# santurini/vsrlab

Hardware: AMD Instinct MI355X
Metric: LR frames/sec fwd+bwd, BasicVSR 4x 540p 7-frame clip, 1->8 MI355X (higher is better)
Workload: dtype bf16; 1 GPU; BasicVSR(mid=64,res_blocks=30,x4) fwd+Charbonnier+bwd+clip+Adam, 540x960->2160x3840, 7-frame clip, 2 clips per GPU (BASELINE configs[1]); clips_per_gpu=2, frames=7, res_blocks=30, parallelism=single GPU, arena=full, train_flow=False, trunk_chains=True

## Files before the change

### vsrlab_amd/csrc/conv_mfma.hip

```cpp
#include <cstdlib>
#include "elt.h"

namespace {

__device__ uint4 g_cm_zero[4];

constexpr int TW = 32;
constexpr int RW = 2;
constexpr int TH = 4 * RW;
constexpr int NTHREADS = 256;

typedef __attribute__((ext_vector_type(4))) unsigned cu32x4_t;
typedef __attribute__((ext_vector_type(8))) unsigned cu32x8_t;
template <typename T> struct RegChunk;
template <> struct RegChunk<bf16_t> { typedef cu32x4_t chunk_t; };
template <> struct RegChunk<float> { typedef cu32x8_t chunk_t; };
__device__ __forceinline__ cu32x4_t reg_chunk3(float a, float b, float c, bf16_t*) {
    union { bf16_t h[8]; cu32x4_t u; } t;
    t.u = cu32x4_t{0u, 0u, 0u, 0u};
    t.h[0] = (bf16_t)a; t.h[1] = (bf16_t)b; t.h[2] = (bf16_t)c;
    return t.u;
}
__device__ __forceinline__ cu32x8_t reg_chunk3(float a, float b, float c, float*) {
    return cu32x8_t{__float_as_uint(a), __float_as_uint(b), __float_as_uint(c), 0u, 0u, 0u, 0u, 0u};
// ... 345 lines not shown
int launch_inst(const ConvArgs& a, hipStream_t st) {
    constexpr int TWH = TW + KS - 1, THH = TH + KS - 1;
    constexpr int CMAX = CA > CB ? CA : CB;
    constexpr int CHB = Elt<T>::CHB;
    constexpr int TPS = conv_taps_per_stage<KS, NSRC>(THH * TWH * (CMAX / 8) * CHB, COUT * (CMAX / 8) * CHB);
    constexpr int LDS = THH * TWH * (CMAX / 8) * CHB + (TPS > 1 ? TPS : 2) * COUT * (CMAX / 8) * CHB;
    static_assert(LDS <= 160 * 1024, "tile does not fit the 160 KiB LDS of a CU");
    auto kern = conv_mfma_kernel<T, KS, NSRC, CA, CB, LP, COUT, EPI>;
    static VsrDevOnce once;
    { const int rc = vsr_set_max_dynamic_lds(once, reinterpret_cast<const void*>(kern), LDS); if (rc != VSR_OK) return rc; }
    dim3 grid(cdiv(a.W, TW), cdiv(a.H, TH), a.N * a.nz);
    hipLaunchKernelGGL(kern, grid, dim3(NTHREADS), LDS, st, a);
    HIP_CHECK_RET(hipGetLastError());
    return VSR_OK;
}

}

#define VSR_CONV_SHAPES(X)                  \
    X(3, 1, 64, 64, false, 64, EPI_NHWC)     \
    X(3, 2, 64, 16, true, 64, EPI_NHWC)      \
    X(3, 1, 16, 16, true, 64, EPI_NHWC)      \
    X(3, 1, 64, 64, false, 32, EPI_PLANAR)   \
    X(3, 4, 64, 64, false, 64, EPI_NHWC)     \
    X(1, 2, 64, 64, false, 64, EPI_NHWC)     \
    X(1, 1, 64, 64, false, 64, EPI_NHWC)     \
    X(7, 1, 16, 16, false, 32, EPI_NHWC)     \
    X(7, 1, 32, 32, false, 64, EPI_NHWC)     \
    X(7, 1, 64, 64, false, 32, EPI_NHWC)     \
    X(7, 1, 32, 32, false, 32, EPI_NHWC)    \
    X(7, 1, 16, 16, false, 32, EPI_PLANAR)   \
     \
    X(3, 1, 16, 16, false, 32, EPI_NHWC)     \
    X(3, 1, 32, 32, false, 32, EPI_NHWC)     \
    X(3, 2, 16, 16, true, 32, EPI_NHWC)      \
    X(3, 2, 32, 16, true, 32, EPI_NHWC)      \
    X(3, 1, 16, 16, true, 32, EPI_NHWC)      \
    X(1, 2, 16, 16, false, 32, EPI_NHWC)     \
    X(1, 2, 32, 32, false, 32, EPI_NHWC)    \
    X(1, 1, 16, 16, false, 32, EPI_NHWC)     \
    X(1, 1, 32, 32, false, 32, EPI_NHWC)    \
    X(3, 4, 16, 16, false, 32, EPI_NHWC)     \
    X(3, 4, 32, 32, false, 32, EPI_NHWC)    \
    X(3, 1, 16, 16, false, 64, EPI_NHWC)     \
    X(3, 1, 32, 32, false, 64, EPI_NHWC)    \
    X(3, 1, 64, 64, false, 32, EPI_NHWC)     \
    X(3, 1, 16, 16, false, 32, EPI_PLANAR)   \
    X(3, 1, 32, 32, false, 32, EPI_PLANAR)

int vsr_launch_conv3x3_c64_persist(const ConvArgs& a, int num_cus, hipStream_t st);
int vsr_launch_c64_to_planar(const ConvArgs& a, hipStream_t st);
int vsr_launch_planar_c64_conv(const ConvArgs& a, hipStream_t st);
int vsr_launch_conv7x7_persist(const ConvArgs& a, int cin, int cop, int epi, int num_cus, hipStream_t st);

static bool vsr_force_generic_conv() { return vsr_env().generic_conv; }

int vsr_launch_conv(int dtype, int ks, int nsrc, int ca, int cb, int last_planar, int cout_t, int epi,
                    const ConvArgs& a, hipStream_t st) {
    if (a.N <= 0 || a.H <= 0 || a.W <= 0 || a.nz < 1 || a.nz > VSR_MAX_Z) return VSR_ERR_BADARG;
    if (dtype == VSR_BF16 && ks == 3 && nsrc == 1 && ca == 64 && cb == 64 && !last_planar && cout_t == 64 && epi == EPI_NHWC &&
        ((a.in_step == 1 && a.src_oy[0] == 0 && a.src_ox[0] == 0 && a.Hs == a.H && a.Ws == a.W) ||
         (a.in_step == 2 && a.Hs == 2 * a.H && a.Ws == 2 * a.W && (unsigned)a.src_oy[0] < 2u && (unsigned)a.src_ox[0] < 2u)) &&
        a.CD == 64 && a.cout_real == 64 &&
        a.src[0] != nullptr && !vsr_force_generic_conv()) {
        const int ps = vsr_launch_conv3x3_c64_persist(a, vsr_num_cus(), st);
        if (ps != VSR_ERR_UNSUPPORTED) return ps;
    }
    if (a.unshuffle) return VSR_ERR_UNSUPPORTED;
    if (dtype == VSR_BF16 && ks == 3 && nsrc == 1 && ca == 64 && cb == 64 && !last_planar && cout_t == 32 && epi == EPI_PLANAR &&
        !vsr_force_generic_conv()) {
        const int ps = vsr_launch_c64_to_planar(a, st);
        if (ps != VSR_ERR_UNSUPPORTED) return ps;
    }
    if (dtype == VSR_BF16 && ks == 3 && nsrc == 1 && last_planar && ca == 16 && cb == 16 && cout_t == 64 && epi == EPI_NHWC && !vsr_force_generic_conv()) {
        const int ps = vsr_launch_planar_c64_conv(a, st);
        if (ps != VSR_ERR_UNSUPPORTED) return ps;
    }
    if (dtype == VSR_BF16 && ks == 7 && nsrc == 1 && ca == cb && !last_planar && !vsr_force_generic_conv()) {
        const int ps = vsr_launch_conv7x7_persist(a, ca, cout_t, epi, vsr_num_cus(), st);
        if (ps != VSR_ERR_UNSUPPORTED) return ps;
    }
#define X(KS, NSRC, CA, CB, LP, COUT, EPI)                                                             \
    if (ks == KS && nsrc == NSRC && ca == CA && cb == CB && (last_planar != 0) == LP && cout_t == COUT && epi == EPI) { \
        if (dtype == VSR_BF16) return launch_inst<bf16_t, KS, NSRC, CA, CB, LP, COUT, EPI>(a, st);    \
        if (dtype == VSR_F32) return launch_inst<float, KS, NSRC, CA, CB, LP, COUT, EPI>(a, st);      \
        return VSR_ERR_BADARG;                                                                        \
    }
    VSR_CONV_SHAPES(X)
#undef X
    return VSR_ERR_UNSUPPORTED;
}
```

### vsrlab_amd/csrc/elementwise.hip

```cpp
#include "elt.h"
#include "kernels.h"

namespace {

__device__ __forceinline__ float warp_coord(float base, float flow, int dim) {
    const float d = (float)(dim - 1 > 1 ? dim - 1 : 1);
    const float g = 2.0f * (base + flow) / d - 1.0f;
    return (g + 1.0f) * 0.5f * (float)(dim - 1);
}

struct WarpSample {
    int x0, y0;
    float wx0, wx1, wy0, wy1;
    float px, py;
    bool in_x, in_y;
};
__device__ __forceinline__ void warp_sample_at(float px, float py, WarpSample& s) {
    const float fx0 = floorf(px), fy0 = floorf(py);
    s.x0 = (int)fx0; s.y0 = (int)fy0;
    s.wx1 = px - fx0; s.wy1 = py - fy0; s.wx0 = 1.f - s.wx1; s.wy0 = 1.f - s.wy1;
}
__device__ __forceinline__ bool warp_floor_fits(float px, float py) {
    return !(fabsf(floorf(px)) > 1e9f || fabsf(floorf(py)) > 1e9f);
}
__device__ __forceinline__ WarpSample warp_sample(int x, int y, float flow_x, float flow_y, int H, int W, int border) {
    WarpSample s;
    float px = warp_coord((float)x, flow_x, W);
    float py = warp_coord((float)y, flow_y, H);
    s.px = px; s.py = py;
    s.in_x = !border || (px >= 0.f && px <= (float)(W - 1)); s.in_y = !border || (py >= 0.f && py <= (float)(H - 1));
    if (border) { px = fminf(fmaxf(px, 0.f), (float)(W - 1)); py = fminf(fmaxf(py, 0.f), (float)(H - 1)); }
    warp_sample_at(px, py, s);
    return s;
}
__device__ __forceinline__ float grad_gate_open(float p, int dim) { return (p <= 0.f || p >= (float)(dim - 1)) ? 0.f : 1.f; }

struct WarpTap { int xi, yi; float wgt; };
__device__ __forceinline__ WarpTap warp_tap(const WarpSample& s, int t) {
    WarpTap p;
    p.xi = s.x0 + (t & 1); p.yi = s.y0 + (t >> 1);
    p.wgt = ((t & 1) ? s.wx1 : s.wx0) * ((t >> 1) ? s.wy1 : s.wy0);
    return p;
}
#define TAP_IN_IMAGE(p, H, W) ((p).xi >= 0 && (p).xi < (W) && (p).yi >= 0 && (p).yi < (H))

template <typename T>
__global__ void warp_fwd_kernel(const T* __restrict__ in, const float* __restrict__ flow, T* __restrict__ out,
                                int N, int H, int W, int C, long long flow_nstride, int border) {
    typedef typename Elt<T>::chunk_t chunk_t;
    const int CP = C / 8;
    const long long total = (long long)N * H * W * CP;
    for (long long idx = (long long)blockIdx.x * blockDim.x + threadIdx.x; idx < total; idx += (long long)gridDim.x * blockDim.x) {
        const int c = (int)(idx % CP);
        const long long pix = idx / CP;
        const int x = (int)(pix % W);
        const int y = (int)((pix / W) % H);
        const int n = (int)(pix / ((long long)W * H));
        const float* fp = flow + (long long)n * flow_nstride + (long long)y * W + x;
        const WarpSample s = warp_sample(x, y, fp[0], fp[(long long)H * W], H, W, border);
        float accv[8];
#pragma unroll
        for (int j = 0; j < 8; ++j) accv[j] = 0.f;
        const T* img = in + (long long)n * pm_image_elems(H, W, C);
#pragma unroll
        for (int t = 0; t < 4; ++t) {
            const WarpTap p = warp_tap(s, t);
            if (TAP_IN_IMAGE(p, H, W)) {
                float f[8];
                unpack8(*reinterpret_cast<const chunk_t*>(img + pm_off(p.yi, p.xi, c, W, C)), f);
#pragma unroll
                for (int j = 0; j < 8; ++j) accv[j] += f[j] * p.wgt;
            }
        }
        chunk_t o;
        pack8(accv, o);
        *reinterpret_cast<chunk_t*>(out + (long long)n * pm_image_elems(H, W, C) + pm_off(y, x, c, W, C)) = o;
    }
}

template <typename T>
__global__ void warp_bwd_kernel(const T* __restrict__ dout, const float* __restrict__ flow, float* __restrict__ dacc,
                                int N, int H, int W, int C, long long flow_nstride, int border) {
    const long long total = (long long)N * H * W * C;
    for (long long idx = (long long)blockIdx.x * blockDim.x + threadIdx.x; idx < total; idx += (long long)gridDim.x * blockDim.x) {
        const int c = (int)(idx % C);
        const long long pix = idx / C;
        const int x = (int)(pix % W);
        const int y = (int)((pix / W) % H);
        const int n = (int)(pix / ((long long)W * H));
        const float* fp = flow + (long long)n * flow_nstride + (long long)y * W + x;
        const WarpSample s = warp_sample(x, y, fp[0], fp[(long long)H * W], H, W, border);
        const float g = (float)dout[(long long)n * pm_image_elems(H, W, C) + pm_off(y, x, c >> 3, W, C) + (c & 7)];
        float* img = dacc + (long long)n * H * W * C;
#pragma unroll
        for (int t = 0; t < 4; ++t) {
            const WarpTap p = warp_tap(s, t);
            if (TAP_IN_IMAGE(p, H, W)) atomicAdd(img + ((long long)p.yi * W + p.xi) * C + c, g * p.wgt);
        }
    }
}

constexpr int GR = 5;
constexpr int GTH = 8, GTW = 32, GCAP = 8;
constexpr int GHH = GTH + 2 * GR, GHW = GTW + 2 * GR;
constexpr double FAR_FX = 17592186044416.0;
constexpr int FAR_BAD = 0x40000000;

__device__ __forceinline__ bool flow_is_far(float fx, float fy) {
    return !(fabsf(fx) <= (float)(GR - 1) && fabsf(fy) <= (float)(GR - 1));
}

template <typename T, int C>
__global__ __launch_bounds__(256) void warp_bwd_gather_kernel(const T* __restrict__ dout, const float* __restrict__ flow, const T* __restrict__ dtop,
                                                              long long* __restrict__ S, const int* __restrict__ far_count, T* __restrict__ out,
                                                              int N, int H, int W, long long flow_nstride) {
    constexpr int CP = C / 8, PPP = 256 / CP;
    typedef typename Elt<T>::chunk_t chunk_t;
    __shared__ float2 pos[GHH * GHW];
    __shared__ unsigned short hit_src[256 * GCAP];
    __shared__ float hit_w[256 * GCAP];
    __shared__ int hit_n[256];
    const int tid = threadIdx.x;
    const int ntx = cdiv(W, GTW), nty = cdiv(H, GTH);
    const int tile = blockIdx.x;
    const int n = tile / (ntx * nty), tr = tile - n * ntx * nty;
    const int ty0 = (tr / ntx) * GTH, tx0 = (tr % ntx) * GTW;
    const float* fbase = flow + (long long)n * flow_nstride;
    const long long img = (long long)n * pm_image_elems(H, W, C);
    for (int i = tid; i < GHH * GHW; i += 256) {
// ... 563 lines not shown
    float4* d4 = reinterpret_cast<float4*>(dsr);
    for (long long i = (long long)blockIdx.x * blockDim.x + threadIdx.x; i < n4; i += (long long)gridDim.x * blockDim.x) {
        const float4 a = s4[i], b = h4[i];
        float4 o;
        float d, r;
        d = a.x - b.x; r = sqrtf(d * d + eps); local += r; o.x = scale * d / r;
        d = a.y - b.y; r = sqrtf(d * d + eps); local += r; o.y = scale * d / r;
        d = a.z - b.z; r = sqrtf(d * d + eps); local += r; o.z = scale * d / r;
        d = a.w - b.w; r = sqrtf(d * d + eps); local += r; o.w = scale * d / r;
        d4[i] = o;
    }
    if (!vec) {
        for (long long i = (long long)blockIdx.x * blockDim.x + threadIdx.x; i < n; i += (long long)gridDim.x * blockDim.x) {
            const float d = sr[i] - hr[i];
            const float r = sqrtf(d * d + eps);
            local += r;
            dsr[i] = scale * d / r;
        }
    } else if (blockIdx.x == 0 && threadIdx.x < (int)(n & 3)) {
        const long long i = (n4 << 2) + threadIdx.x;
        const float d = sr[i] - hr[i];
        const float r = sqrtf(d * d + eps);
        local += r;
        dsr[i] = scale * d / r;
    }
    for (int o = 32; o > 0; o >>= 1) local += __shfl_down(local, o, 64);
    if ((threadIdx.x & 63) == 0) red[threadIdx.x >> 6] = local;
    __syncthreads();
    if (threadIdx.x == 0) partial[blockIdx.x] = ((red[0] + red[1]) + (red[2] + red[3])) * scale;
}
__global__ void charbonnier_sum_kernel(const float* __restrict__ partial, int nblocks, float* __restrict__ loss) {
    __shared__ float red[256];
    float s = 0.f;
    for (int i = threadIdx.x; i < nblocks; i += 256) s += partial[i];
    red[threadIdx.x] = s;
    __syncthreads();
    for (int o = 128; o > 0; o >>= 1) {
        if (threadIdx.x < o) red[threadIdx.x] += red[threadIdx.x + o];
        __syncthreads();
    }
    if (threadIdx.x == 0) loss[0] = red[0];
}

}

#define DISPATCH_T(dtype, CALL)                              \
    if ((dtype) == VSR_BF16) { typedef bf16_t T; CALL; }     \
    else if ((dtype) == VSR_F32) { typedef float T; CALL; }  \
    else return VSR_ERR_BADARG;

int vsr_launch_warp_fwd(int dtype, const void* in, const float* flow, void* out, int N, int H, int W, int C,
                        long long flow_nstride, hipStream_t st, int border) {
    if (C % 8) return VSR_ERR_BADARG;
    const long long total = (long long)N * H * W * (C / 8);
    DISPATCH_T(dtype, hipLaunchKernelGGL(warp_fwd_kernel<T>, dim3(grid_for(total)), dim3(256), 0, st, (const T*)in, flow, (T*)out, N, H, W, C, flow_nstride, border));
    HIP_CHECK_RET(hipGetLastError());
    return VSR_OK;
}

int vsr_launch_warp_bwd(int dtype, const void* dout, const float* flow, float* dacc, int N, int H, int W, int C,
                        long long flow_nstride, hipStream_t st, int border) {
    const long long total = (long long)N * H * W * C;
    DISPATCH_T(dtype, hipLaunchKernelGGL(warp_bwd_kernel<T>, dim3(grid_for(total)), dim3(256), 0, st, (const T*)dout, flow, dacc, N, H, W, C, flow_nstride, border));
    HIP_CHECK_RET(hipGetLastError());
    return VSR_OK;
}

template <int C>
static int warp_bwd_gather_c(int dtype, const void* dout, const float* flow, const void* dtop, long long* S, int* far_count, void* out,
                             int N, int H, int W, long long flow_nstride, hipStream_t st) {
    const long long npix = (long long)N * H * W;
    const int tiles = N * cdiv(H, GTH) * cdiv(W, GTW);
    long long gb = (npix + 255) / 256;
    if (gb > 256 * 16) gb = 256 * 16;
    if (gb < 1) gb = 1;
    DISPATCH_T(dtype, hipLaunchKernelGGL((warp_bwd_far_kernel<T, C>), dim3((int)gb), dim3(256), 0, st, (const T*)dout, flow, S, far_count, N, H, W, flow_nstride));
    DISPATCH_T(dtype, hipLaunchKernelGGL((warp_bwd_gather_kernel<T, C>), dim3(tiles), dim3(256), 0, st, (const T*)dout, flow, (const T*)dtop, S,
                                         (const int*)far_count, (T*)out, N, H, W, flow_nstride));
    HIP_CHECK_RET(hipGetLastError());
    return VSR_OK;
}
int vsr_launch_warp_bwd_gather(int dtype, const void* dout, const float* flow, const void* dtop, long long* S, int* far_count, void* out,
                               int N, int H, int W, int C, long long flow_nstride, hipStream_t st) {
    if (!dout || !flow || !S || !far_count || !out) return VSR_ERR_BADARG;
    if (C == 64) return warp_bwd_gather_c<64>(dtype, dout, flow, dtop, S, far_count, out, N, H, W, flow_nstride, st);
    if (C == 32) return warp_bwd_gather_c<32>(dtype, dout, flow, dtop, S, far_count, out, N, H, W, flow_nstride, st);
    if (C == 16) return warp_bwd_gather_c<16>(dtype, dout, flow, dtop, S, far_count, out, N, H, W, flow_nstride, st);
    return VSR_ERR_UNSUPPORTED;
}

int vsr_launch_add_cast(int dtype, const void* a, const float* s, void* out, int N, int H, int W, int C, hipStream_t st) {
    const long long total = (long long)N * H * W * (C / 8);
    DISPATCH_T(dtype, hipLaunchKernelGGL(add_cast_kernel<T>, dim3(grid_for(total)), dim3(256), 0, st, (const T*)a, s, (T*)out, N, H, W, C));
    HIP_CHECK_RET(hipGetLastError());
    return VSR_OK;
}

int vsr_launch_planar_to_pm(int dtype, const float* in, void* out, int N, int Cin, int H, int W, int C, hipStream_t st) {
    const long long total = (long long)N * H * W * C;
    DISPATCH_T(dtype, hipLaunchKernelGGL(planar_to_pm_kernel<T>, dim3(grid_for(total)), dim3(256), 0, st, in, (T*)out, N, Cin, H, W, C));
    HIP_CHECK_RET(hipGetLastError());
    return VSR_OK;
}

int vsr_launch_pm_to_planar(int dtype, const void* in, float* out, int N, int Cout, int H, int W, int C, hipStream_t st) {
    const long long total = (long long)N * Cout * H * W;
    DISPATCH_T(dtype, hipLaunchKernelGGL(pm_to_planar_kernel<T>, dim3(grid_for(total)), dim3(256), 0, st, (const T*)in, out, N, Cout, H, W, C));
    HIP_CHECK_RET(hipGetLastError());
// ... 121 lines not shown
```

### vsrlab_amd/csrc/engine.hip

```cpp
#include <vector>
#include "recipes.h"
#include "spynet_engine.h"

namespace {

struct Plan {
    VsrBasicVSRDesc d = {};
    int C = 64, CO = 64;
    bool sb = false;
    bool bwd = false, flowgrad = false;
    bool diet = false;
    int rb = 0, n = 0, t = 0, h = 0, w = 0, dtype = VSR_F32;
    int scale = 4, ups = 2;
    bool unsh = false;
    size_t es = 4;
    size_t px1 = 0;
    size_t s_elems = 0;
    size_t stem_w[2] = {}, stem_wd[2] = {}, stem_b[2] = {};
    std::vector<size_t> blk_w[2], blk_wd[2], blk_b[2];
    size_t point_w = 0, point_wd = 0, point_b = 0;
    size_t up_w[2] = {}, up_wd[2] = {}, up_b[2] = {};
    size_t last0_w = 0, last0_wd = 0, last0_b = 0, last2_w = 0, last2_wd = 0, last2_b = 0;
    SpyPlan spy;
    size_t flows = 0;
// ... 243 lines not shown
              chain_off(p.blk_w[dir][2 * b]), chain_off(p.blk_b[dir][2 * b]), CHAIN_RELU};
        ChainLayer& l2 = a.layer[2 * b + 1];
        l2 = {chain_off(p.aoff(dir, i, b)), chain_off(p.xoff(dir, i, b + 1)), chain_off(p.xoff(dir, i, b)), 0xffffffffu, 0xffffffffu,
              chain_off(p.blk_w[dir][2 * b + 1]), chain_off(p.blk_b[dir][2 * b + 1]), CHAIN_SKIP};
    }
    return chain_launch(a, c.st);
}
int trunk_chain_backward(const Ctx& c, const Plan& p, int dir, int i) {
    ChainArgs a = {};
    a.base = c.ws; a.sync = (unsigned*)c.at(p.chain_sync[dir]); a.N = p.n; a.H = p.h; a.W = p.w;
    int L = 0;
    for (int b = p.rb - 1; b >= 0; --b) {
        a.layer[L++] = {chain_off(p.dxoff(dir, i, b + 1)), chain_off(p.g1off(dir, i, b)), 0xffffffffu, chain_off(p.sboff(dir, i, b)), 0xffffffffu,
                        chain_off(p.blk_wd[dir][2 * b + 1]), 0xffffffffu, CHAIN_MASK};
        if (b > 0)
            a.layer[L++] = {chain_off(p.g1off(dir, i, b)), chain_off(p.dxoff(dir, i, b)), chain_off(p.dxoff(dir, i, b + 1)), 0xffffffffu, 0xffffffffu,
                            chain_off(p.blk_wd[dir][2 * b]), 0xffffffffu, CHAIN_SKIP};
    }
    a.nlayers = L;
    return chain_launch(a, c.st);
}

int trunk_forward(const Ctx& c, const Plan& p, int dir, int i, const void* warped, const float* lrs) {
    const int n = p.n, h = p.h, w = p.w, rb = p.rb;
    void* x = p.bwd ? c.at(p.xoff(dir, i, 0)) : c.at(p.feat[dir][i]);
    {
        CK(c.stem(true, warped, lrs + (size_t)i * 3 * h * w, (long long)p.t * 3 * h * w, c.at(p.stem_w[dir]), c.fat(p.stem_b[dir]), x, ACT_LEAKY, 0.f, n, h, w));
        if (p.sb) CK(vsr_launch_sign_bits_c64(x, c.at(p.SBX0[dir][i]), n, h, w, c.st));
    }
    if (chain_on(p)) return trunk_chain_forward(c, p, dir, i);
    for (int b = 0; b < rb; ++b) {
        void* act = p.bwd ? c.at(p.aoff(dir, i, b)) : c.at(p.scratchA[dir]);
        void* xn = p.bwd ? c.at(p.xoff(dir, i, b + 1)) : x;
        CK(c.conv(3, x, c.at(p.blk_w[dir][2 * b]), c.fat(p.blk_b[dir][2 * b]), act, ACT_RELU, nullptr, nullptr, 0, n, h, w,
                    p.sb ? c.at(p.sboff(dir, i, b)) : nullptr));
        CK(c.conv(3, act, c.at(p.blk_w[dir][2 * b + 1]), c.fat(p.blk_b[dir][2 * b + 1]), xn, ACT_NONE, x, nullptr, 0, n, h, w));
        x = xn;
    }
    return VSR_OK;
}

int last0_forward(const Ctx& c, const Plan& p, int i, void* sign_out) {
    const int S = p.scale;
    if (p.C == 64)
        return c.conv(3, c.at(p.U1[i]), c.at(p.last0_w), c.fat(p.last0_b), c.at(p.C0[i]), ACT_LEAKY, nullptr, nullptr, 0, p.n, S * p.h, S * p.w, sign_out);
    ConvArgs a = conv_args(p.n, S * p.h, S * p.w, c.C);
    a.src[0] = c.at(p.U1[i]); a.wpack = c.at(p.last0_w); a.bias = c.fat(p.last0_b); a.dst[0] = c.at(p.C0[i]); a.act = ACT_LEAKY;
    a.CD = 64; a.cout_real = 64; a.dst_nstride = pm_image_elems(S * p.h, S * p.w, 64);
    return vsr_launch_conv(c.dtype, 3, 1, p.C, p.C, 0, 64, EPI_NHWC, a, c.st);
}

int recon_forward(const Ctx& c, const Plan& p, int i, const float* lrs, float* sr) {
    const int n = p.n, h = p.h, w = p.w;
    CK(c.point_conv(c.at(p.feat[0][i]), c.at(p.feat[1][i]), c.at(p.point_w), c.fat(p.point_b), c.at(p.Pt[i]), n, h, w));
    if (p.sb) CK(vsr_launch_sign_bits_c64(c.at(p.Pt[i]), c.at(p.SBPt[i]), n, h, w, c.st));
    const int S = p.scale;
    CK(c.conv_ps(c.at(p.Pt[i]), c.at(p.up_w[0]), c.fat(p.up_b[0]), c.at(p.U0[i]), n, h, w));
    if (p.ups == 2) CK(c.conv_ps(c.at(p.U0[i]), c.at(p.up_w[1]), c.fat(p.up_b[1]), c.at(p.U1[i]), n, 2 * h, 2 * w));
    CK(last0_forward(c, p, i, p.sb ? c.at(p.SBC0[i]) : nullptr));
    {
        ConvArgs a = conv_args(n, S * h, S * w, c.C);
        a.src_nstride[0] = pm_image_elems(S * h, S * w, 64);
        a.src[0] = c.at(p.C0[i]); a.wpack = c.at(p.last2_w); a.bias = c.fat(p.last2_b); a.cout_real = 3;
        a.dst[0] = sr + (size_t)i * 3 * S * S * h * w; a.dst_nstride = (long long)p.t * 3 * S * S * h * w;
        a.base_lr = lrs + (size_t)i * 3 * h * w; a.base_nstride = (long long)p.t * 3 * h * w; a.base_h = h; a.base_w = w; a.base_scale = S;
        CK(vsr_launch_conv(c.dtype, 3, 1, 64, 64, 0, 32, EPI_PLANAR, a, c.st));
    }
    return VSR_OK;
}

const float* flow_ptr(const Ctx& c, const Plan& p, int forward, int i) {
    return c.fat(p.flows) + ((size_t)forward * p.n * (p.t - 1) + i) * 2 * p.h * p.w;
}

struct Helper { hipStream_t s = nullptr; hipEvent_t fork = nullptr, join = nullptr; int dev = -1; };
int get_helper(Helper** out) {
    thread_local Helper hp[16];
    int dev = 0;
    HIP_CHECK_RET(hipGetDevice(&dev));
    if (dev < 0 || dev >= 16) return VSR_ERR_UNSUPPORTED;
    Helper& x = hp[dev];
    if (!x.s) {
        HIP_CHECK_RET(hipStreamCreateWithFlags(&x.s, hipStreamNonBlocking));
        HIP_CHECK_RET(hipEventCreateWithFlags(&x.fork, hipEventDisableTiming));
        HIP_CHECK_RET(hipEventCreateWithFlags(&x.join, hipEventDisableTiming));
        x.dev = dev;
    }
    *out = &x;
    return VSR_OK;
}
bool single_stream() { return vsr_env().single_stream; }
struct Fork {
    hipStream_t main; Helper* h; bool active = false;
    int begin(bool fork = true) {
        if (single_stream() || !fork) return VSR_OK;
        CK(get_helper(&h));
        HIP_CHECK_RET(hipEventRecord(h->fork, main));
        HIP_CHECK_RET(hipStreamWaitEvent(h->s, h->fork, 0));
        active = true;
        return VSR_OK;
    }
    hipStream_t side() const { return active ? h->s : main; }
    int end() {
        if (!active) return VSR_OK;
        active = false;
        HIP_CHECK_RET(hipEventRecord(h->join, h->s));
        HIP_CHECK_RET(hipStreamWaitEvent(main, h->join, 0));
        return VSR_OK;
// ... 328 lines not shown
```

### vsrlab_amd/csrc/recipes.h

```cpp
#pragma once
#include <vector>
#include "host.h"

inline constexpr int NSPY = 5;
inline constexpr int SPY_CI[NSPY] = {8, 32, 64, 32, 16};
inline constexpr int SPY_CO[NSPY] = {32, 64, 32, 16, 2};
inline constexpr int SPY_CIP[NSPY] = {16, 32, 64, 32, 16};
inline constexpr int SPY_COP[NSPY] = {32, 64, 32, 32, 32};
inline constexpr int SPY_CD[NSPY] = {32, 64, 32, 16, 0};
inline constexpr int SPY_DK[NSPY] = {32, 64, 32, 16, 16};
inline constexpr int SPY_DROWS[NSPY] = {32, 32, 64, 32, 32};

struct Ctx {
    char* ws;
    hipStream_t st;
    int dtype;
    int C, CO;
    size_t es;
    float* slab;
    mutable std::vector<VsrPackDesc>* batch = nullptr;
    Ctx(char* ws_, hipStream_t st_, int dtype_, int C_ = 64, float* slab_ = nullptr)
        : ws(ws_), st(st_), dtype(dtype_), C(C_), CO(C_ < 32 ? 32 : C_), es(esize(dtype_)), slab(slab_) {}
    void* at(size_t off) const { return ws + off; }
    const float* fat(size_t off) const { return reinterpret_cast<const float*>(ws + off); }
// ... 50 lines not shown
                if (z == 3) { a.aux[0] = aux; a.mask_mode = mask; a.sign_bits[0] = aux ? sign_bits : nullptr; }
                int rc = vsr_launch_conv(dtype, 3, 1, 64, 64, 0, 64, EPI_NHWC, a, st);
                if (rc != VSR_OK) return rc;
            }
            return VSR_OK;
        }
        ConvArgs a = conv_args(N, H, W, C);
        a.nz = 1; a.in_step = 2; a.Hs = 2 * H; a.Ws = 2 * W;
        for (int s = 0; s < 4; ++s) { a.src[s] = dy; a.src_oy[s] = s >> 1; a.src_ox[s] = s & 1; a.src_nstride[s] = pm_image_elems(2 * H, 2 * W, C); }
        a.wpack = wpackd; a.dst[0] = dx; a.aux[0] = aux; a.mask_mode = mask;
        return vsr_launch_conv(dtype, 3, 4, C, C, 0, CO, EPI_NHWC, a, st);
    }
    int ps_wgrads(const void* const* x, const void* const* dy, int nseg, bool dy_planes, int N, int H, int W, float* gw, float* gb, int accumulate) const {
        for (int z = 0; z < 4; ++z) {
            WgradArgs a = wg_base(N, H, W, C, C);
            a.nseg = nseg;
            for (int i = 0; i < nseg; ++i) {
                a.x[i] = x[i];
                a.dy[i] = dy_planes ? (const char*)dy[i] + (size_t)z * plane_elems(N, 2 * H, 2 * W) * es : dy[i];
            }
            if (!dy_planes) { a.dy_step = 2; a.dy_oy = z >> 1; a.dy_ox = z & 1; a.Hy = 2 * H; a.Wy = 2 * W; a.dy_nstride = pm_image_elems(2 * H, 2 * W, C); }
            CK(wgrad(a, {3, C, false, C, false}, {C, C, gw, C, 0, 4, z, gb, accumulate}));
        }
        return VSR_OK;
    }

    int pack_stem(const float* w, void* dst, bool cat) const {
        const int I_total = cat ? C + 3 : 3;
        if (cat) CK(pack(w, dst, 9, CO, C, C, C, I_total, 3, 1, 0, 0));
        return pack(w, (char*)dst + (cat ? (size_t)9 * CO * C * es : 0), 9, CO, 16, C, 3, I_total, 0, 1, 0, 0);
    }
    int pack_stem_dgrad(const float* w, void* dst) const { return pack(w, dst, 9, CO, C, C, C, C + 3, 3, 1, 0, 1); }
    int pack_stem_dlr(const float* w, void* dst, bool cat) const { return pack(w, dst, 9, 32, C, 3, C, cat ? C + 3 : 3, 0, 1, 0, 1); }
    int stem(bool cat, const void* feat, const float* lr, long long lr_nstride, const void* wpack, const float* bias, void* y, int act, float slope,
             int N, int H, int W) const {
        ConvArgs a = conv_args(N, H, W, C);
        a.wpack = wpack; a.bias = bias; a.dst[0] = y; a.act = act; a.leaky_slope = slope;
        a.src[cat ? 1 : 0] = lr; a.src_nstride[cat ? 1 : 0] = lr_nstride;
        if (!cat) return vsr_launch_conv(dtype, 3, 1, 16, 16, 1, CO, EPI_NHWC, a, st);
        a.src[0] = feat;
        return vsr_launch_conv(dtype, 3, 2, C, 16, 1, CO, EPI_NHWC, a, st);
    }
    int stem_wgrads(bool cat, WgradArgs& a_lr, WgradArgs& a_feat, float* gw, float* gb, int accumulate) const {
        const int I_total = cat ? C + 3 : 3;
        CK(wgrad(a_lr, {3, 16, true, C, false}, {C, 3, gw, I_total, 0, 1, 0, gb, accumulate}));
        if (cat && a_feat.nseg) CK(wgrad_cc(3, a_feat, gw, I_total, 3, nullptr, accumulate));
        return VSR_OK;
    }

    int pack_point(const float* w, void* dst, int mode) const {
        for (int s = 0; s < 2; ++s) CK(pack(w, (char*)dst + (size_t)s * CO * C * es, 1, CO, C, C, C, 2 * C, s * C, 1, 0, mode));
        return VSR_OK;
    }
    int point_conv(const void* xa, const void* xb, const void* wpack, const float* bias, void* y, int N, int H, int W) const {
        ConvArgs a = conv_args(N, H, W, C);
        a.src[0] = xa; a.src[1] = xb;
        a.wpack = wpack; a.bias = bias; a.dst[0] = y; a.act = ACT_LEAKY;
        return vsr_launch_conv(dtype, 1, 2, C, C, 0, CO, EPI_NHWC, a, st);
    }
    int point_dgrad(const void* dy, const void* wpackd, void* da, void* db, int N, int H, int W) const {
        ConvArgs a = conv_args(N, H, W, C);
        a.src[0] = dy; a.wpack = wpackd; a.w_zstride = CO * C; a.nz = 2;
        a.dst[0] = da; a.dst[1] = db;
        return vsr_launch_conv(dtype, 1, 1, C, C, 0, CO, EPI_NHWC, a, st);
    }

    int pack_spy(int j, const float* w, void* dst, int mode) const {
        if (mode == 0) return pack(w, dst, 49, SPY_COP[j], SPY_CIP[j], SPY_CO[j], SPY_CI[j], SPY_CI[j], 0, 1, 0, 0);
        return pack(w, dst, 49, SPY_DROWS[j], SPY_DK[j], SPY_CI[j], SPY_CO[j], SPY_CI[j], 0, 1, 0, 1);
    }
    int spy_conv(int j, const void* x, const void* wpack, const float* bias, void* y, int act, float slope, const float* pres, int N, int H, int W) const {
        ConvArgs a = conv_args(N, H, W, SPY_CD[j]);
        a.src[0] = x; a.src_nstride[0] = pm_image_elems(H, W, SPY_CIP[j]);
        a.wpack = wpack; a.bias = bias; a.act = act; a.leaky_slope = slope; a.cout_real = SPY_CO[j]; a.dst[0] = y;
        if (j < NSPY - 1) return vsr_launch_conv(dtype, 7, 1, SPY_CIP[j], SPY_CIP[j], 0, SPY_COP[j], EPI_NHWC, a, st);
        a.dst_nstride = (long long)2 * H * W; a.pres = pres;
        return vsr_launch_conv(dtype, 7, 1, 16, 16, 0, 32, EPI_PLANAR, a, st);
    }
    int spy_dgrad(int j, const void* dy, const void* wpackd, void* dx, const void* aux, int N, int H, int W) const {
        const int CI = SPY_CIP[j], DK = SPY_DK[j];
        ConvArgs a = conv_args(N, H, W, CI);
        a.src[0] = dy; a.src_nstride[0] = pm_image_elems(H, W, DK);
        a.wpack = wpackd; a.dst[0] = dx; a.cout_real = j == 0 ? 8 : CI;
        if (aux) { a.aux[0] = aux; a.mask_mode = MASK_RELU; }
        return vsr_launch_conv(dtype, 7, 1, DK, DK, 0, SPY_DROWS[j], EPI_NHWC, a, st);
    }
    int spy_wgrad(int j, const void* x, const void* dy, int N, int H, int W, float* gw, float* gb, int accumulate) const {
        const int CI = SPY_CIP[j], DK = SPY_DK[j];
        const int nhalf = (dtype == VSR_F32 && CI == 64) ? 2 : 1;
        for (int hf = 0; hf < nhalf; ++hf) {
            WgradArgs a = wg_base(N, H, W, CI, DK);
            a.x[0] = x; a.dy[0] = dy;
            const int cx = CI / nhalf;
            if (nhalf == 2) { a.x_ctotal = CI; a.x_coff = hf * (cx / 8); }
            const int cin_real = nhalf == 2 ? cx : SPY_CI[j];
            CK(wgrad(a, {7, cx, false, DK, false}, {SPY_CO[j], cin_real, gw, SPY_CI[j], hf * cx, 1, 0, hf == 0 ? gb : nullptr, accumulate}));
        }
        return VSR_OK;
    }

    int wgrad(WgradArgs& a, const WgradShape& s, const WgradDst& d, bool even = true) const { return wgrad_run(st, dtype, slab, a, s, d, even); }
    int wgrad_cc(int ks, WgradArgs& a, float* gw, int I_total, int i_off, float* gb, int accumulate) const {
        return wgrad(a, {ks, C, false, C, false}, {C, C, gw, I_total, i_off, 1, 0, gb, accumulate});
    }

    int pack_cc(int ks, const float* w, void* dst, int mode) const { return pack(w, dst, ks * ks, CO, C, C, C, C, 0, 1, 0, mode); }
    int pack(const float* w, void* dst, int KK, int RP, int CPd, int r_real, int c_real, int I_total, int i_off, int o_mul,
             int o_add, int mode) const {
        return pack_any(dtype, w, dst, KK, RP, CPd, r_real, c_real, I_total, i_off, o_mul, o_add, mode);
    }
    int pack_bias(const float* b, void* dst, int nreal, int o_mul = 1, int o_add = 0) const {
// ... 15 lines not shown
```

Before: 59.21 LR frames/s.

## Add dedicated 1x1 c64 MFMA kernel with fused sign bits; tile warp_fwd per pixel

Adds a persistent 1x1 conv kernel for 64-channel bf16 that keeps weight fragments in registers and can write the sign-bit words for the backward leaky ReLU in its epilogue. This removes the separate sign_bits pass over the point-conv output and replaces the generic templated 1x1 path for both the forward conv and the dgrad. The warp forward kernel is also restructured so each thread owns one pixel, computes its bilinear taps once and loops over channel chunks, instead of recomputing flow sampling for every 8-channel chunk. The risks are register pressure from the fixed waves_per_eu setting and extra correctness surface in the sign-word layout.

```diff
diff --git a/vsrlab_amd/csrc/conv_mfma.hip b/vsrlab_amd/csrc/conv_mfma.hip
--- a/vsrlab_amd/csrc/conv_mfma.hip
+++ b/vsrlab_amd/csrc/conv_mfma.hip
@@ -421,6 +421,7 @@
 int vsr_launch_c64_to_planar(const ConvArgs& a, hipStream_t st);
 int vsr_launch_planar_c64_conv(const ConvArgs& a, hipStream_t st);
 int vsr_launch_conv7x7_persist(const ConvArgs& a, int cin, int cop, int epi, int num_cus, hipStream_t st);
+int vsr_launch_point_c64(const ConvArgs& a, int nsrc, int num_cus, hipStream_t st);
 
 static bool vsr_force_generic_conv() { return vsr_env().generic_conv; }
 
@@ -449,6 +450,10 @@
         const int ps = vsr_launch_conv7x7_persist(a, ca, cout_t, epi, vsr_num_cus(), st);
         if (ps != VSR_ERR_UNSUPPORTED) return ps;
     }
+    if (dtype == VSR_BF16 && ks == 1 && ca == 64 && cb == 64 && !last_planar && cout_t == 64 && epi == EPI_NHWC && !vsr_force_generic_conv()) {
+        const int ps = vsr_launch_point_c64(a, nsrc, vsr_num_cus(), st);
+        if (ps != VSR_ERR_UNSUPPORTED) return ps;
+    }
 #define X(KS, NSRC, CA, CB, LP, COUT, EPI)                                                             \
     if (ks == KS && nsrc == NSRC && ca == CA && cb == CB && (last_planar != 0) == LP && cout_t == COUT && epi == EPI) { \
         if (dtype == VSR_BF16) return launch_inst<bf16_t, KS, NSRC, CA, CB, LP, COUT, EPI>(a, st);    \
diff --git a/vsrlab_amd/csrc/elementwise.hip b/vsrlab_amd/csrc/elementwise.hip
--- a/vsrlab_amd/csrc/elementwise.hip
+++ b/vsrlab_amd/csrc/elementwise.hip
@@ -44,37 +44,55 @@
 }
 #define TAP_IN_IMAGE(p, H, W) ((p).xi >= 0 && (p).xi < (W) && (p).yi >= 0 && (p).yi < (H))
 
-template <typename T>
-__global__ void warp_fwd_kernel(const T* __restrict__ in, const float* __restrict__ flow, T* __restrict__ out,
-                                int N, int H, int W, int C, long long flow_nstride, int border) {
+constexpr int WF_TH = 8;
+template <typename T, int CB>
+__global__ __launch_bounds__(256) void warp_fwd_kernel(const T* __restrict__ in, const float* __restrict__ flow, T* __restrict__ out,
+                                                       int N, int H, int W, int C, long long flow_nstride, int border) {
     typedef typename Elt<T>::chunk_t chunk_t;
+    const int ws = pm_ws(W), per = cdiv(H, WF_TH) * ws;
+    const int n = blockIdx.x / per, r = blockIdx.x - n * per;
+    const int ty = r / ws, seg = r - ty * ws;
+    const int y = ty * WF_TH + (threadIdx.x >> 5), x = seg * 32 + (threadIdx.x & 31);
+    if (y >= H || x >= W) return;
+    const float* fp = flow + (long long)n * flow_nstride + (long long)y * W + x;
+    const WarpSample s = warp_sample(x, y, fp[0], fp[(long long)H * W], H, W, border);
+    const T* img = in + (long long)n * pm_image_elems(H, W, C);
+    long long toff[4];
+    float twgt[4];
+    bool tin[4];
+#pragma unroll
+    for (int t = 0; t < 4; ++t) {
+        const WarpTap p = warp_tap(s, t);
+        tin[t] = TAP_IN_IMAGE(p, H, W);
+        toff[t] = tin[t] ? pm_off(p.yi, p.xi, 0, W, C) : 0;
+        twgt[t] = p.wgt;
+    }
+    T* o = out + (long long)n * pm_image_elems(H, W, C) + pm_off(y, x, 0, W, C);
     const int CP = C / 8;
-    const long long total = (long long)N * H * W * CP;
-    for (long long idx = (long long)blockIdx.x * blockDim.x + threadIdx.x; idx < total; idx += (long long)gridDim.x * blockDim.x) {
-        const int c = (int)(idx % CP);
-        const long long pix = idx / CP;
-        const int x = (int)(pix % W);
-        const int y = (int)((pix / W) % H);
-        const int n = (int)(pix / ((long long)W * H));
-        const float* fp = flow + (long long)n * flow_nstride + (long long)y * W + x;
-        const WarpSample s = warp_sample(x, y, fp[0], fp[(long long)H * W], H, W, border);
-        float accv[8];
-#pragma unroll
-        for (int j = 0; j < 8; ++j) accv[j] = 0.f;
-        const T* img = in + (long long)n * pm_image_elems(H, W, C);
-#pragma unroll
-        for (int t = 0; t < 4; ++t) {
-            const WarpTap p = warp_tap(s, t);
-            if (TAP_IN_IMAGE(p, H, W)) {
-                float f[8];
-                unpack8(*reinterpret_cast<const chunk_t*>(img + pm_off(p.yi, p.xi, c, W, C)), f);
-#pragma unroll
-                for (int j = 0; j < 8; ++j) accv[j] += f[j] * p.wgt;
+    for (int c0 = 0; c0 < CP; c0 += CB) {
+        chunk_t v[CB][4];
+#pragma unroll
+        for (int k = 0; k < CB; ++k)
+#pragma unroll
+            for (int t = 0; t < 4; ++t) v[k][t] = *reinterpret_cast<const chunk_t*>(img + toff[t] + (long long)(c0 + k) * 256);
+#pragma unroll
+        for (int k = 0; k < CB; ++k) {
+            float accv[8];
+#pragma unroll
+            for (int j = 0; j < 8; ++j) accv[j] = 0.f;
+#pragma unroll
+            for (int t = 0; t < 4; ++t) {
+                if (tin[t]) {
+                    float f[8];
+                    unpack8(v[k][t], f);
+#pragma unroll
+                    for (int j = 0; j < 8; ++j) accv[j] += f[j] * twgt[t];
+                }
             }
-        }
-        chunk_t o;
-        pack8(accv, o);
-        *reinterpret_cast<chunk_t*>(out + (long long)n * pm_image_elems(H, W, C) + pm_off(y, x, c, W, C)) = o;
+            chunk_t ov;
+            pack8(accv, ov);
+            *reinterpret_cast<chunk_t*>(o + (long long)(c0 + k) * 256) = ov;
+        }
     }
 }
 
@@ -744,8 +762,13 @@
 int vsr_launch_warp_fwd(int dtype, const void* in, const float* flow, void* out, int N, int H, int W, int C,
                         long long flow_nstride, hipStream_t st, int border) {
     if (C % 8) return VSR_ERR_BADARG;
-    const long long total = (long long)N * H * W * (C / 8);
-    DISPATCH_T(dtype, hipLaunchKernelGGL(warp_fwd_kernel<T>, dim3(grid_for(total)), dim3(256), 0, st, (const T*)in, flow, (T*)out, N, H, W, C, flow_nstride, border));
+    if (C < 8 || N < 1 || H < 1 || W < 1) return VSR_OK;
+    const long long tiles = (long long)N * cdiv(H, WF_TH) * pm_ws(W);
+    if (tiles > 0x7fffffffLL) return VSR_ERR_UNSUPPORTED;
+    const int CP = C / 8;
+#define WARP_FWD(CB) DISPATCH_T(dtype, hipLaunchKernelGGL((warp_fwd_kernel<T, CB>), dim3((unsigned)tiles), dim3(256), 0, st, (const T*)in, flow, (T*)out, N, H, W, C, flow_nstride, border))
+    if (CP % 4 == 0) { WARP_FWD(4); } else if (CP % 2 == 0) { WARP_FWD(2); } else { WARP_FWD(1); }
+#undef WARP_FWD
     HIP_CHECK_RET(hipGetLastError());
     return VSR_OK;
 }
diff --git a/vsrlab_amd/csrc/engine.hip b/vsrlab_amd/csrc/engine.hip
--- a/vsrlab_amd/csrc/engine.hip
+++ b/vsrlab_amd/csrc/engine.hip
@@ -319,8 +319,7 @@
 
 int recon_forward(const Ctx& c, const Plan& p, int i, const float* lrs, float* sr) {
     const int n = p.n, h = p.h, w = p.w;
-    CK(c.point_conv(c.at(p.feat[0][i]), c.at(p.feat[1][i]), c.at(p.point_w), c.fat(p.point_b), c.at(p.Pt[i]), n, h, w));
-    if (p.sb) CK(vsr_launch_sign_bits_c64(c.at(p.Pt[i]), c.at(p.SBPt[i]), n, h, w, c.st));
+    CK(c.point_conv(c.at(p.feat[0][i]), c.at(p.feat[1][i]), c.at(p.point_w), c.fat(p.point_b), c.at(p.Pt[i]), n, h, w, p.sb ? c.at(p.SBPt[i]) : nullptr));
     const int S = p.scale;
     CK(c.conv_ps(c.at(p.Pt[i]), c.at(p.up_w[0]), c.fat(p.up_b[0]), c.at(p.U0[i]), n, h, w));
     if (p.ups == 2) CK(c.conv_ps(c.at(p.U0[i]), c.at(p.up_w[1]), c.fat(p.up_b[1]), c.at(p.U1[i]), n, 2 * h, 2 * w));
diff --git a/vsrlab_amd/csrc/lr_stream.hip b/vsrlab_amd/csrc/lr_stream.hip
--- /dev/null
+++ b/vsrlab_amd/csrc/lr_stream.hip
@@ -0,0 +1,154 @@
+#include <cstddef>
+#include "elt.h"
+#include "kernels.h"
+#include "conv3x3_c64_tile.h"
+
+namespace {
+
+constexpr int LS_RW = 2;
+static_assert(PTW == 32 && PTH == 4 * LS_RW, "the tile of the sign words");
+constexpr int LS_SIGN_BYTES = LS_RW * 8 * 512;
+
+__device__ __forceinline__ float ls_bf_lo(unsigned w) { return __uint_as_float(w << 16); }
+__device__ __forceinline__ float ls_bf_hi(unsigned w) { return __uint_as_float(w & 0xffff0000u); }
+
+template <int NSRC, int NZ, bool SIGN>
+__global__ __launch_bounds__(256) __attribute__((amdgpu_waves_per_eu(3, 3))) void point_c64_kernel(const ConvArgs a, int tiles) {
+    static_assert(NSRC * NZ == 2 && (!SIGN || NZ == 1), "16 weight fragments per lane");
+    __shared__ __attribute__((aligned(16))) char sgn[SIGN ? 4 * LS_SIGN_BYTES : 16];
+    const int lane = threadIdx.x & 63, wave = threadIdx.x >> 6;
+    const int l31 = lane & 31, h = lane >> 5;
+    const int ntx = pm_ws(a.W), nty = cdiv(a.H, PTH);
+    const float slope = vsr_slope(a.leaky_slope);
+
+    bf16x8_t af[NZ][NSRC][4][2];
+#pragma unroll
+    for (int z = 0; z < NZ; ++z)
+#pragma unroll
+        for (int s = 0; s < NSRC; ++s)
+#pragma unroll
+            for (int ks = 0; ks < 4; ++ks)
+#pragma unroll
+                for (int cb = 0; cb < 2; ++cb)
+                    af[z][s][ks][cb] = *reinterpret_cast<const bf16x8_t*>(reinterpret_cast<const bf16_t*>(a.wpack) + (long long)z * a.w_zstride +
+                                                                          s * 64 * 64 + ((cb * 32 + l31) * 8 + 2 * ks + h) * 8);
+
+    for (int tile = blockIdx.x; tile < tiles; tile += gridDim.x) {
+        const int n = tile / (ntx * nty), r = tile - n * ntx * nty;
+        const int ty = r / ntx, tx = r - ty * ntx;
+        const int x = tx * PTW + l31;
+        const int y0 = ty * PTH + wave * LS_RW;
+        long long poff[LS_RW];
+        bool ok[LS_RW];
+#pragma unroll
+        for (int rw = 0; rw < LS_RW; ++rw) {
+            ok[rw] = x < a.W && y0 + rw < a.H;
+            poff[rw] = ok[rw] ? pm_off(y0 + rw, x, 0, a.W, 64) : 0;
+        }
+        bf16x8_t bf[NSRC][4][LS_RW];
+#pragma unroll
+        for (int s = 0; s < NSRC; ++s) {
+            const bf16_t* base = reinterpret_cast<const bf16_t*>(a.src[s]) + (long long)n * a.src_nstride[s] + h * 256;
+#pragma unroll
+            for (int ks = 0; ks < 4; ++ks)
+#pragma unroll
+                for (int rw = 0; rw < LS_RW; ++rw) bf[s][ks][rw] = *reinterpret_cast<const bf16x8_t*>(base + poff[rw] + 2 * ks * 256);
+        }
+#pragma unroll
+        for (int z = 0; z < NZ; ++z) {
+#pragma unroll
+            for (int rw = 0; rw < LS_RW; ++rw) {
+                f32x16_t acc[2];
+#pragma unroll
+                for (int cb = 0; cb < 2; ++cb)
+#pragma unroll
+                    for (int i = 0; i < 16; ++i) acc[cb][i] = 0.f;
+#pragma unroll
+                for (int s = 0; s < NSRC; ++s)
+#pragma unroll
+                    for (int ks = 0; ks < 4; ++ks)
+#pragma unroll
+                        for (int cb = 0; cb < 2; ++cb) mma(acc[cb], af[z][s][ks][cb], bf[s][ks][rw]);
+
+                if (!ok[rw]) continue;
+                bf16_t* dst = reinterpret_cast<bf16_t*>(a.dst[z]) + (long long)n * a.dst_nstride + poff[rw];
+#pragma unroll
+                for (int cb = 0; cb < 2; ++cb)
+#pragma unroll
+                    for (int g = 0; g < 4; ++g) {
+                        const int co = cb * 32 + 8 * g + 4 * h;
+                        float v[4];
+#pragma unroll
+                        for (int j = 0; j < 4; ++j) v[j] = acc[cb][4 * g + j];
+                        if (a.bias) {
+                            const float4 b = *reinterpret_cast<const float4*>(a.bias + (long long)z * a.bias_zstride + co);
+                            v[0] += b.x; v[1] += b.y; v[2] += b.z; v[3] += b.w;
+                        }
+                        if (a.act == ACT_RELU) {
+#pragma unroll
+                            for (int j = 0; j < 4; ++j) v[j] = v[j] > 0.f ? v[j] : 0.f;
+                        } else if (a.act == ACT_LEAKY) {
+#pragma unroll
+                            for (int j = 0; j < 4; ++j) v[j] = v[j] > 0.f ? v[j] : slope * v[j];
+                        }
+                        Vec4<bf16_t> o;
+#pragma unroll
+                        for (int j = 0; j < 4; ++j) o.v[j] = (bf16_t)v[j];
+                        *reinterpret_cast<Vec4<bf16_t>*>(dst + (co >> 3) * 256 + (co & 7)) = o;
+                        if (SIGN) *reinterpret_cast<Vec4<bf16_t>*>(sgn + wave * LS_SIGN_BYTES + (rw * 8 + (co >> 3)) * 512 + l31 * 16 + (co & 7) * 2) = o;
+                    }
+            }
+        }
+        if (SIGN) {
+            __builtin_amdgcn_fence(__ATOMIC_RELEASE, "wavefront");
+            __builtin_amdgcn_wave_barrier();
+            __builtin_amdgcn_fence(__ATOMIC_ACQUIRE, "wavefront");
+            const int l15 = lane & 15, q = lane >> 4;
+            const int pxl = PM_LANE_PIXEL(l15);
+            unsigned out[2] = {0u, 0u};
+#pragma unroll
+            for (int nb = 0; nb < 4; ++nb) {
+                const int yy = y0 + (nb >> 1), xx = tx * PTW + (nb & 1) * 16 + pxl;
+                if (yy < a.H && xx < a.W) {
+#pragma unroll
+                    for (int k = 0; k < 2; ++k) {
+                        const uint4 v = *reinterpret_cast<const uint4*>(sgn + wave * LS_SIGN_BYTES + ((nb >> 1) * 8 + 4 * k + q) * 512 + ((nb & 1) * 16 + pxl) * 16);
+                        const unsigned vw[4] = {v.x, v.y, v.z, v.w};
+#pragma unroll
+                        for (int jj = 0; jj < 4; ++jj)
+                            out[k] |= ((ls_bf_lo(vw[jj]) > 0.f ? 1u : 0u) | (ls_bf_hi(vw[jj]) > 0.f ? 0x10000u : 0u)) << (4 * nb + jj);
+                    }
+                }
+            }
+            reinterpret_cast<uint2*>(a.sign_out[0])[c64_sign_word(tile, wave, lane)] = make_uint2(out[0], out[1]);
+            __builtin_amdgcn_fence(__ATOMIC_RELEASE, "wavefront");
+            __builtin_amdgcn_wave_barrier();
+        }
+    }
+}
+
+template <int NSRC, int NZ, bool SIGN>
+int launch_point(const ConvArgs& a, int num_cus, hipStream_t st) {
+    const long long tiles = (long long)a.N * cdiv(a.H, PTH) * pm_ws(a.W);
+    if (tiles > 0x7fffffffLL) return VSR_ERR_UNSUPPORTED;
+    const long long gx = tiles < 3LL * num_cus ? tiles : 3LL * num_cus;
+    hipLaunchKernelGGL((point_c64_kernel<NSRC, NZ, SIGN>), dim3((unsigned)gx), dim3(256), 0, st, a, (int)tiles);
+    HIP_CHECK_RET(hipGetLastError());
+    return VSR_OK;
+}
+
+}
+
+static_assert(sizeof(ConvArgs) == 448 && offsetof(ConvArgs, sign_out) == 360 && offsetof(ConvArgs, unshuffle_plane) == 440,
+              "tests/test_lr_stream_gpu.py reaches the sign-word epilogue through vsr_launch_conv with a ctypes mirror of ConvArgs: keep it in step");
+int vsr_launch_point_c64(const ConvArgs& a, int nsrc, int num_cus, hipStream_t st) {
+    if (a.in_step != 1 || a.Hs != a.H || a.Ws != a.W || a.out_step != 1 || a.Hd != a.H || a.Wd != a.W || a.CD != 64 || a.cout_real != 64 ||
+        a.unshuffle || !a.wpack)
+        return VSR_ERR_UNSUPPORTED;
+    if (!((nsrc == 2 && a.nz == 1) || (nsrc == 1 && a.nz == 2))) return VSR_ERR_UNSUPPORTED;
+    for (int s = 0; s < nsrc; ++s) if (!a.src[s] || a.src_oy[s] || a.src_ox[s]) return VSR_ERR_UNSUPPORTED;
+    for (int z = 0; z < a.nz; ++z) if (!a.dst[z] || a.res[z] || a.aux[z] || a.out_oy[z] || a.out_ox[z]) return VSR_ERR_UNSUPPORTED;
+    if (a.sign_out[0] && (nsrc != 2 || a.act == ACT_NONE)) return VSR_ERR_UNSUPPORTED;
+    if (nsrc == 1) return launch_point<1, 2, false>(a, num_cus, st);
+    return a.sign_out[0] ? launch_point<2, 1, true>(a, num_cus, st) : launch_point<2, 1, false>(a, num_cus, st);
+}
diff --git a/vsrlab_amd/csrc/recipes.h b/vsrlab_amd/csrc/recipes.h
--- a/vsrlab_amd/csrc/recipes.h
+++ b/vsrlab_amd/csrc/recipes.h
@@ -126,11 +126,15 @@
         for (int s = 0; s < 2; ++s) CK(pack(w, (char*)dst + (size_t)s * CO * C * es, 1, CO, C, C, C, 2 * C, s * C, 1, 0, mode));
         return VSR_OK;
     }
-    int point_conv(const void* xa, const void* xb, const void* wpack, const float* bias, void* y, int N, int H, int W) const {
+    int point_conv(const void* xa, const void* xb, const void* wpack, const float* bias, void* y, int N, int H, int W, void* sign_out = nullptr) const {
+        if (sign_out && (dtype != VSR_BF16 || C != 64)) return VSR_ERR_UNSUPPORTED;
         ConvArgs a = conv_args(N, H, W, C);
         a.src[0] = xa; a.src[1] = xb;
         a.wpack = wpack; a.bias = bias; a.dst[0] = y; a.act = ACT_LEAKY;
-        return vsr_launch_conv(dtype, 1, 2, C, C, 0, CO, EPI_NHWC, a, st);
+        a.sign_out[0] = sign_out;
+        const int rc = vsr_launch_conv(dtype, 1, 2, C, C, 0, CO, EPI_NHWC, a, st);
+        if (rc == VSR_OK && sign_out && vsr_env().generic_conv) return vsr_launch_sign_bits_c64(y, sign_out, N, H, W, st);
+        return rc;
     }
     int point_dgrad(const void* dy, const void* wpackd, void* da, void* db, int N, int H, int W) const {
         ConvArgs a = conv_args(N, H, W, C);
```

New measurement: 59.46 LR frames/s, median of 6. No clear change (+0.4%).
